# olegroshka/vae-channel-dynamics

Measured on AMD Instinct MI355X. Metric: images/sec SDXL-VAE train step @256x256 (tracking on), higher is better.
Workload: dtype f32

## Files before the change

### vae-channel-dynamics_amd/csrc/igemm.hip

```cpp
#include "bf16_frag.h"
#include <algorithm>
#include <stdlib.h>
#include <type_traits>

#include "launchers.h"

namespace {

struct LanePos {
  int lr, lh, trq, trp, trh;
};
__device__ __forceinline__ LanePos lane_pos(int lane) { return LanePos{lane & 31, lane >> 5, (lane & 15) >> 2, lane & 3, (lane >> 4) & 1}; }

struct F32 {
  typedef float elem;
  typedef f32x4 raw4;
  typedef f32x4 frag;
  typedef unsigned off_t;
  static constexpr int BK_ROWS = 32, BK_WGRAD = 32;
  static constexpr int KG = 8;
  static constexpr int PAD_K = 4, PAD_T = 4;
  static constexpr bool SETPRIO = true;
  static constexpr bool PAIR16 = false;
  static constexpr bool flag(int32_t) { return false; }

  static __device__ __forceinline__ raw4 load4(__amdgpu_buffer_rsrc_t rs, unsigned, bool ok, int row, int ld, int c) {
    return VAE_BUF_LOAD4(rs, oob_unless(ok, ((unsigned)row * (unsigned)ld + (unsigned)c) * 4u));
  }
  static __device__ __forceinline__ f32x4 to_f32(raw4 r, bool) { return r; }
  static __device__ __forceinline__ void put4(elem* d, f32x4 v) { *reinterpret_cast<f32x4*>(d) = v; }
  static __device__ __forceinline__ void put4_stored(elem* d, raw4, f32x4 v, bool) { put4(d, v); }
  static __device__ __forceinline__ frag frag_k(const elem* p) { return *reinterpret_cast<const f32x4*>(p); }
  static __device__ __forceinline__ frag frag_t(const elem* tile, int ld, int kg, LanePos l, int col0) {
    frag v;
#pragma unroll
    for (int j = 0; j < 4; ++j) v[j] = tile[(kg * 8 + l.lh * 4 + j) * ld + col0 + l.lr];
    return v;
  }
  template <int MI, int NI>
  static __device__ __forceinline__ void frags_tt(frag* a, frag* b, const elem* sA, int ldA, int colA, const elem* sB, int ldB, int colB, int kg, LanePos l) {
#pragma unroll
    for (int j = 0; j < 4; ++j) {
      const int k = kg * 8 + l.lh * 4 + j;
#pragma unroll
      for (int mi = 0; mi < MI; ++mi) a[mi][j] = sA[k * ldA + colA + mi * 32 + l.lr];
#pragma unroll
      for (int ni = 0; ni < NI; ++ni) b[ni][j] = sB[k * ldB + colB + ni * 32 + l.lr];
    }
  }
  template <int MI, int NI>
  static __device__ __forceinline__ void mma(f32x16 (&acc)[MI][NI], const frag* a, const frag* b) {
#pragma unroll
    for (int j = 0; j < 4; ++j)
#pragma unroll
      for (int mi = 0; mi < MI; ++mi)
#pragma unroll
        for (int ni = 0; ni < NI; ++ni) acc[mi][ni] = __builtin_amdgcn_mfma_f32_32x32x2f32(a[mi][j], b[ni][j], acc[mi][ni], 0, 0, 0);
  }
  static __device__ __forceinline__ off_t out_off(bool ok, int orow, int ldc, int col) {
    return ok ? ((unsigned)orow * (unsigned)ldc + (unsigned)col) * 4u : BUF_OOB;
  }
  static __device__ __forceinline__ bool inside(off_t o) { return o != BUF_OOB; }
  static __device__ __forceinline__ float load1(__amdgpu_buffer_rsrc_t rs, bool, off_t o) {
    return __builtin_bit_cast(float, __builtin_amdgcn_raw_buffer_load_b32(rs, o, 0, 0));
  }
  static __device__ __forceinline__ void store1(__amdgpu_buffer_rsrc_t rs, bool, off_t o, float v) {
    __builtin_amdgcn_raw_buffer_store_b32(__builtin_bit_cast(unsigned, v), rs, o, 0, 0);
  }
};

struct BF16 {
  typedef u16 elem;
  typedef uint4 raw4;
  typedef bf16x8 frag;
  typedef int off_t;
  static constexpr int BK_ROWS = 64, BK_WGRAD = 32;
  static constexpr int KG = 16;
  static constexpr int PAD_K = 8, PAD_T = 32;
  static constexpr bool SETPRIO = false;
  static constexpr bool PAIR16 = true;
  static __device__ __forceinline__ bool flag(int32_t v) { return v != 0; }

  static __device__ __forceinline__ raw4 load4(__amdgpu_buffer_rsrc_t rs, unsigned esize, bool ok, int row, int ld, int c) {
    return buf_load4_raw(rs, esize, neg_unless(ok, row * ld + c));
  }
  static __device__ __forceinline__ f32x4 to_f32(raw4 r, bool bf) { return raw4_to_f32(r, bf); }
  static __device__ __forceinline__ void put4(elem* d, f32x4 v) { *reinterpret_cast<uint2*>(d) = pack4(v); }
  static __device__ __forceinline__ void put4_stored(elem* d, raw4 r, f32x4 v, bool bf) {
    *reinterpret_cast<uint2*>(d) = bf ? uint2{r.x, r.y} : pack4(v);
  }
  static __device__ __forceinline__ frag frag_k(const elem* p) { return frag_direct(p); }
  static __device__ __forceinline__ frag frag_t(const elem* tile, int ld, int kg, LanePos l, int col0) {
    return frag_tr(tile + (kg * 16 + l.lh * 8 + l.trq) * ld + col0 + l.trh * 16 + l.trp * 4, ld);
  }
  template <int MI, int NI>
  static __device__ __forceinline__ void frags_tt(frag* a, frag* b, const elem* sA, int ldA, int colA, const elem* sB, int ldB, int colB, int kg, LanePos l) {
#pragma unroll
    for (int mi = 0; mi < MI; ++mi) a[mi] = frag_t(sA, ldA, kg, l, colA + mi * 32);
#pragma unroll
    for (int ni = 0; ni < NI; ++ni) b[ni] = frag_t(sB, ldB, kg, l, colB + ni * 32);
  }
  template <int MI, int NI>
  static __device__ __forceinline__ void mma(f32x16 (&acc)[MI][NI], const frag* a, const frag* b) {
#pragma unroll
    for (int mi = 0; mi < MI; ++mi)
#pragma unroll
      for (int ni = 0; ni < NI; ++ni) acc[mi][ni] = __builtin_amdgcn_mfma_f32_32x32x16_bf16(a[mi], b[ni], acc[mi][ni], 0, 0, 0);
  }
  static __device__ __forceinline__ off_t out_off(bool ok, int orow, int ldc, int col) { return ok ? orow * ldc + col : -1; }
  static __device__ __forceinline__ bool inside(off_t o) { return o >= 0; }
  static __device__ __forceinline__ float load1(__amdgpu_buffer_rsrc_t rs, bool bf, off_t o) { return buf_load1_elem(rs, bf, o); }
  static __device__ __forceinline__ void store1(__amdgpu_buffer_rsrc_t rs, bool bf, off_t o, float v) { buf_store1_elem(rs, bf, o, v); }

  static __device__ __forceinline__ bool pair16(const vae_igemm_args& p, bool cbf, bool rbf, const char* C) {
    return cbf && (p.N % 2 == 0) && (p.ldc % 2 == 0) && (p.res == nullptr || rbf) && p.track == nullptr && ((reinterpret_cast<uintptr_t>(C) & 3u) == 0);
  }
  template <int MI, int NI, class RowPixel>
  static __device__ __forceinline__ void store_pairs(const vae_igemm_args& p, const f32x16 (&acc)[MI][NI], int ni, __amdgpu_buffer_rsrc_t rsC,
                                                     __amdgpu_buffer_rsrc_t rsR, int col, bool colok, int m0, int trow0, int lh, bool s2c,
                                                     RowPixel row_pixel) {
    const bool odd = col & 1;
    const float b0 = (p.bias && colok) ? p.bias[col & ~1] : 0.f, b1 = (p.bias && colok) ? p.bias[col | 1] : 0.f;
#pragma unroll
    for (int mi = 0; mi < MI; ++mi) {
      unsigned o16[8], rr[8];
#pragma unroll
      for (int j = 0; j < 8; ++j) {
        const int r = 2 * j + (odd ? 1 : 0);
        const int row = trow0 + mi * 32 + (r & 3) + 8 * (r >> 2) + 4 * lh;
        int orow = row;
        if (s2c) {
          int b, y, x;
          row_pixel(row < p.M ? row : m0, b, y, x);
          orow = (b * p.g.Ho + y) * p.g.Wo + x;
        }
        o16[j] = (colok && row < p.M) ? (unsigned)(orow * p.ldc + (col & ~1)) * 2u : BUF_OOB;
        rr[j] = 0u;
      }
      if (p.res) {
#pragma unroll
        for (int j = 0; j < 8; ++j) rr[j] = __builtin_amdgcn_raw_buffer_load_b32(rsR, o16[j], 0, 0);
      }
#pragma unroll
      for (int j = 0; j < 8; ++j) {
        const float a0 = p.alpha * acc[mi][ni][2 * j], a1 = p.alpha * acc[mi][ni][2 * j + 1];
        const float recv = lane_xor1(odd ? a0 : a1);
        typedef __bf16 bf16x2_t __attribute__((ext_vector_type(2)));
        bf16x2_t h;
        h[0] = (__bf16)((odd ? recv : a0) + b0 + __builtin_bit_cast(float, rr[j] << 16));
        h[1] = (__bf16)((odd ? a1 : recv) + b1 + __builtin_bit_cast(float, rr[j] & 0xffff0000u));
        __builtin_amdgcn_raw_buffer_store_b32(__builtin_bit_cast(unsigned, h), rsC, o16[j], 0, 0);
      }
    }
  }
};

template <int MI, int NI>
__device__ __forceinline__ void zero_acc(f32x16 (&acc)[MI][NI]) {
#pragma unroll
  for (int mi = 0; mi < MI; ++mi)
#pragma unroll
    for (int ni = 0; ni < NI; ++ni)
#pragma unroll
      for (int r = 0; r < 16; ++r) acc[mi][ni][r] = 0.f;
}

template <class P, int BM, int BN, int WM, int WN, bool BKM, bool VEC, int XF>
__device__ __forceinline__ void rows_body(const vae_igemm_args& p) {
  typedef typename P::elem elem;
  constexpr int BK = P::BK_ROWS;
  constexpr int NT = 64 * WM * WN;
  constexpr int KQ = BK / 4;
  constexpr int RP = NT / KQ;
  constexpr int LDA = BK + P::PAD_K;
  constexpr int LDB = BKM ? (BN + P::PAD_T) : (BK + P::PAD_K);
  constexpr int SA = BM * LDA;
  constexpr int SB = BKM ? BK * LDB : BN * LDB;
  constexpr int STAGE = SA + SB;
  constexpr int SS = (XF != VAE_XF_NONE) ? 2 * SS_HALF * (4 / (int)sizeof(elem)) : 0;
  constexpr int TM = BM / WM, TN = BN / WN, MI = TM / 32, NI = TN / 32;
  constexpr int AR = BM / RP;
  constexpr int NQ = BN / 4, KR = NT / NQ;
  constexpr int BR = BKM ? (BK / KR) : (BN / RP);
  static_assert(AR >= 1 && BR >= 1 && TM % 32 == 0 && TN % 32 == 0 && (BK / P::KG == 2 || BK / P::KG == 4), "tile/wave layout");
  __shared__ __attribute__((aligned(16))) elem smem[2 * STAGE + SS];
  float* sS = reinterpret_cast<float*>(smem + 2 * STAGE);

  const int tid = threadIdx.x, lane = tid & 63, wave = tid >> 6;
  const int wm = wave / WN, wn = wave % WN;
  const LanePos lp = lane_pos(lane);
  const int lr = lp.lr, lh = lp.lh;
  const int tilesN = (p.N + BN - 1) / BN;
  const int tm = blockIdx.x / tilesN, tn = blockIdx.x % tilesN;
  const int m0 = tm * BM, n0 = tn * BN;
  const int z = blockIdx.z;
  const vae_conv_geom g = p.g;
  const SrcMap smap = make_srcmap(g);
  const bool abf = P::flag(p.a_bf16), cbf = P::flag(p.out_bf16), rbf = P::flag(p.res_bf16);
  const unsigned esA = abf ? 2u : 4u;
  const char* __restrict__ A = reinterpret_cast<const char*>(p.A) + (int64_t)z * p.sAb * esA;
  const float* __restrict__ W = p.W + (int64_t)z * p.sWb;
  const int hw = g.Ho * g.Wo;

  const bool s2c = (g.mode == VAE_MODE_DGRAD_S2);
  const int hh = g.Ho >> 1, wh = g.Wo >> 1;
  const int cls_rows = s2c ? p.M >> 2 : 1;
  const int cls = s2c ? m0 / cls_rows : 0;
  const int cpy = cls >> 1, cpx = cls & 1;
  const int nkw = s2c ? (cpx ? 1 : 2) : 3;
  const int ntaps = s2c ? (cpy ? 1 : 2) * nkw : g.taps;
  auto row_pixel = [&](int m, int& b, int& y, int& x) {
    if (s2c) {
      const int r = m - cls * cls_rows;
      b = r / (hh * wh);
      const int rem = r - b * (hh * wh);
      const int i = rem / wh;
      y = 2 * i + cpy;
      x = 2 * (rem - i * wh) + cpx;
    } else {
      b = m / hw;
      const int rem = m - b * hw;
      y = rem / g.Wo;
      x = rem - y * g.Wo;
    }
  };

  const int b_base = s2c ? (m0 - cls * cls_rows) / (hh * wh) : m0 / hw;
  const size_t img = (size_t)g.Hs * g.Ws * g.Cs;
  const size_t abytes = (size_t)(g.B - b_base) * img * esA, wbytes = (size_t)(BKM ? (int64_t)p.K * p.sk : (int64_t)p.N * p.sn) * 4u;
  const auto rsA = VAE_BUF_RSRC(A + (int64_t)b_base * img * esA, abytes < BUF_MAX ? abytes : BUF_MAX);
  const auto rsW = VAE_BUF_RSRC(W, wbytes < BUF_MAX ? wbytes : BUF_MAX);

  const int k4 = tid % KQ, r0 = tid / KQ;
  const int n4 = tid % NQ, kq = tid / NQ;
  int rb[AR], ry[AR], rx[AR];
#pragma unroll
  for (int i = 0; i < AR; ++i) {
    const int m = m0 + r0 + RP * i;
    if (m < p.M) {
      row_pixel(m, rb[i], ry[i], rx[i]);
    } else {
      rb[i] = -1; ry[i] = 0; rx[i] = 0;
    }
  }

  const int b_lo = m0 / hw;
  if (XF != VAE_XF_NONE) {
    const int b_hi = (min(p.M, m0 + BM) - 1) / hw;
    const int nent = min((b_hi - b_lo + 1) * p.K, SS_HALF);
    for (int i = tid; i < nent; i += NT) {
      const int j = i / p.K, c = i - j * p.K;
      sS[i] = p.scale[(int64_t)(b_lo + j) * g.Cs + c];
      sS[SS_HALF + i] = p.shift[(int64_t)(b_lo + j) * g.Cs + c];
    }
  }

  f32x16 acc[MI][NI];
  zero_acc(acc);

  const int kchunks = (p.K + BK - 1) / BK;
  const int steps = ntaps * kchunks;

  typename P::raw4 ra[AR];
  f32x4 rw[BR];
  int a_b[AR];
  int reg_c0 = 0;

  auto load_regs = [&](int s) {
    const int ord = s / kchunks;
    const int c0 = (s - ord * kchunks) * BK;
    reg_c0 = c0;
    int kh, kw;
    if (s2c) {
      const int a = ord / nkw;
      kh = cpy ? 1 : 2 * a;
      kw = cpx ? 1 : 2 * (ord - a * nkw);
    } else {
      kh = (g.taps == 9) ? ord / 3 : 0;
      kw = (g.taps == 9) ? ord - kh * 3 : 0;
    }
    const int tap = kh * 3 + kw;
    const int c = c0 + k4 * 4;
#pragma unroll
    for (int i = 0; i < AR; ++i) {
      int sy = 0, sx = 0;
      const bool ok = src_pixel(smap, ry[i], rx[i], kh, kw, sy, sx) && (rb[i] >= 0);
      if constexpr (VEC) ra[i] = P::load4(rsA, esA, ok && c < p.K, ((rb[i] - b_base) * g.Hs + sy) * g.Ws + sx, g.Cs, c);
      else ra[i] = load4s(p.A + (int64_t)z * p.sAb + (((int64_t)rb[i] * g.Hs + sy) * g.Ws + sx) * g.Cs + c, ok, c, p.K);
      a_b[i] = ok ? rb[i] : -1;
    }
    if (!BKM) {
#pragma unroll
      for (int i = 0; i < BR; ++i) {
        const int n = n0 + r0 + RP * i;
        if constexpr (VEC) rw[i] = VAE_BUF_LOAD4(rsW, oob_unless(n < p.N && c < p.K, ((unsigned)n * (unsigned)p.sn + (unsigned)tap * (unsigned)p.st + (unsigned)c) * 4u));
        else rw[i] = load4s(W + (int64_t)n * p.sn + (int64_t)tap * p.st + c, n < p.N, c, p.K);
      }
    } else {
#pragma unroll
      for (int i = 0; i < BR; ++i) {
        const int k = c0 + kq + KR * i;
        const int n = n0 + n4 * 4;
        if constexpr (VEC) rw[i] = VAE_BUF_LOAD4(rsW, oob_unless(k < p.K && n < p.N, ((unsigned)k * (unsigned)p.sk + (unsigned)tap * (unsigned)p.st + (unsigned)n) * 4u));
        else rw[i] = load4s(W + (int64_t)k * p.sk + (int64_t)tap * p.st + n, k < p.K, n, p.N);
      }
    }
  };
  auto store_lds = [&](elem* sA, elem* sB) {
    const int c = reg_c0 + k4 * 4;
#pragma unroll
    for (int i = 0; i < AR; ++i) {
      f32x4 v = P::to_f32(ra[i], abf);
      if (XF != VAE_XF_NONE) {
        const bool ok = (a_b[i] >= 0) && (c < p.K);
        const int o = ok ? (a_b[i] - b_lo) * p.K + c : 0;
        v = xform4_tab<XF>(v, sS + o, sS + SS_HALF + o, ok);
      }
      P::put4(&sA[(r0 + RP * i) * LDA + k4 * 4], v);
    }
#pragma unroll
    for (int i = 0; i < BR; ++i) {
      if (!BKM) P::put4(&sB[(r0 + RP * i) * LDB + k4 * 4], rw[i]);
      else P::put4(&sB[(kq + KR * i) * LDB + n4 * 4], rw[i]);
    }
  };
  typename P::frag fa[2][MI], fb[2][NI];
  auto fetch = [&](const elem* sA, const elem* sB, int kg, typename P::frag* a, typename P::frag* b) {
#pragma unroll
    for (int mi = 0; mi < MI; ++mi) a[mi] = P::frag_k(&sA[(wm * TM + mi * 32 + lr) * LDA + kg * P::KG + lh * (P::KG / 2)]);
#pragma unroll
    for (int ni = 0; ni < NI; ++ni) {
      if (!BKM) b[ni] = P::frag_k(&sB[(wn * TN + ni * 32 + lr) * LDB + kg * P::KG + lh * (P::KG / 2)]);
      else b[ni] = P::frag_t(sB, LDB, kg, lp, wn * TN + ni * 32);
    }
  };
  constexpr int NKG = BK / P::KG;
  auto compute = [&](const elem* sA, const elem* sB, int kg) {
    if (kg + 1 < NKG) fetch(sA, sB, kg + 1, fa[(kg + 1) & 1], fb[(kg + 1) & 1]);
    __builtin_amdgcn_sched_barrier(0);
    if (P::SETPRIO) __builtin_amdgcn_s_setprio(1);
    P::mma(acc, fa[kg & 1], fb[kg & 1]);
    if (P::SETPRIO) __builtin_amdgcn_s_setprio(0);
    __builtin_amdgcn_sched_barrier(0);
  };
  load_regs(0);
  __syncthreads();
  store_lds(smem, smem + SA);
  if (steps > 1) load_regs(1);
  __syncthreads();
  for (int s = 0; s < steps; ++s) {
    const elem* cA = smem + (s & 1) * STAGE;
    const elem* cB = cA + SA;
    fetch(cA, cB, 0, fa[0], fb[0]);
    compute(cA, cB, 0);
    if (NKG == 4) compute(cA, cB, 1);
    if (s + 1 < steps) {
      elem* nA = smem + ((s + 1) & 1) * STAGE;
      store_lds(nA, nA + SA);
      if (s + 2 < steps) load_regs(s + 2);
    }
    compute(cA, cB, NKG / 2);
    if (NKG == 4) compute(cA, cB, 3);
    __syncthreads();
  }

  const unsigned esC = cbf ? 2u : 4u, esR = rbf ? 2u : 4u;
  char* __restrict__ C = reinterpret_cast<char*>(p.C) + (int64_t)z * p.sCb * esC;
  const auto rsC = VAE_BUF_RSRC(C, (size_t)p.M * p.ldc * esC);
  const auto rsR = VAE_BUF_RSRC(p.res ? reinterpret_cast<const char*>(p.res) + (int64_t)z * p.sCb * esR : C, (size_t)p.M * p.ldc * (p.res ? esR : esC));
  float tsum[NI];
#pragma unroll
  for (int ni = 0; ni < NI; ++ni) tsum[ni] = 0.f;
  bool pair16 = false;
  if constexpr (P::PAIR16) pair16 = P::pair16(p, cbf, rbf, C);
#pragma unroll
  for (int ni = 0; ni < NI; ++ni) {
    const int col = n0 + wn * TN + ni * 32 + lr;
    const bool colok = col < p.N;
    const float bv = (p.bias && colok) ? p.bias[col] : 0.f;
    if constexpr (P::PAIR16) {
      if (pair16) {
        P::store_pairs(p, acc, ni, rsC, rsR, col, colok, m0, m0 + wm * TM, lh, s2c, row_pixel);
        continue;
      }
    }
#pragma unroll
    for (int mi = 0; mi < MI; ++mi) {
      typename P::off_t off[16];
      float rv[16];
#pragma unroll
      for (int r = 0; r < 16; ++r) {
        const int row = m0 + wm * TM + mi * 32 + (r & 3) + 8 * (r >> 2) + 4 * lh;
        int orow = row;
        if (s2c) {
          int b, y, x;
          row_pixel(row < p.M ? row : m0, b, y, x);
          orow = (b * g.Ho + y) * g.Wo + x;
        }
        off[r] = P::out_off(colok && row < p.M, orow, p.ldc, col);
        rv[r] = 0.f;
      }
      if (p.res) {
#pragma unroll
        for (int r = 0; r < 16; ++r) rv[r] = P::load1(rsR, rbf, off[r]);
      }
#pragma unroll
      for (int r = 0; r < 16; ++r) {
        const float v = p.alpha * acc[mi][ni][r] + bv + rv[r];
        P::store1(rsC, cbf, off[r], v);
        tsum[ni] += P::inside(off[r]) ? fabsf(v) : 0.f;
      }
    }
  }
  if (p.track && z == 0) {
    float* red = reinterpret_cast<float*>(smem);
#pragma unroll
    for (int ni = 0; ni < NI; ++ni) {
      const float s2 = tsum[ni] + __shfl_xor(tsum[ni], 32, 64);
      if (lh == 0) red[wm * BN + wn * TN + ni * 32 + lr] = s2;
    }
    __syncthreads();
    if (tid < BN) {
      float t = 0.f;
#pragma unroll
      for (int w = 0; w < WM; ++w) t += red[w * BN + tid];
      if (n0 + tid < p.N) p.track[(int64_t)tm * p.N + n0 + tid] = t;
    }
  }
}

template <class P, int BM, int BN, int WM, int WN, bool VEC, int XF>
__device__ __forceinline__ void wgrad_body(const vae_wgrad_args& p) {
  typedef typename P::elem elem;
  constexpr int BK = P::BK_WGRAD;
  constexpr int NT = 64 * WM * WN;
  constexpr int LDA = BM + P::PAD_T, LDB = BN + P::PAD_T;
  constexpr int SA = BK * LDA, SB = BK * LDB;
  constexpr int STAGE = SA + SB;
  constexpr int SS = (XF != VAE_XF_NONE) ? 2 * SS_HALF * (4 / (int)sizeof(elem)) : 0;
  constexpr int TM = BM / WM, TN = BN / WN, MI = TM / 32, NI = TN / 32;
  constexpr int AQ = BM / 4, AKR = NT / AQ, AI = BK / AKR;
  constexpr int BQ = BN / 4, BKR = NT / BQ, BI = BK / BKR;
  static_assert(AI >= 1 && BI >= 1 && TM % 32 == 0 && TN % 32 == 0 && (BK / P::KG == 2 || BK / P::KG == 4), "tile/wave layout");
  __shared__ __attribute__((aligned(16))) elem smem[2 * STAGE + SS];
  float* sS = reinterpret_cast<float*>(smem + 2 * STAGE);

  const int tid = threadIdx.x, lane = tid & 63, wave = tid >> 6;
  const int wm = wave / WN, wn = wave % WN;
  const LanePos lp = lane_pos(lane);
  const int lr = lp.lr, lh = lp.lh;
  const int tilesN = (p.N + BN - 1) / BN;
  const int tm = blockIdx.x / tilesN, tn = blockIdx.x % tilesN;
  const int m0 = tm * BM, n0 = tn * BN;
  const int tap = blockIdx.y / p.nsplit, split = blockIdx.y % p.nsplit;
  const int z = blockIdx.z;
  const vae_conv_geom g = p.g;
  const SrcMap smap = make_srcmap(g);
  const int kh = (g.taps == 9) ? tap / 3 : 0, kw = (g.taps == 9) ? tap - kh * 3 : 0;
  const bool ybf = P::flag(p.y_bf16), xbf = P::flag(p.x_bf16);
  const unsigned esY = ybf ? 2u : 4u, esX = xbf ? 2u : 4u;
  const char* __restrict__ dY = reinterpret_cast<const char*>(p.dY) + (int64_t)z * p.sYb * esY;
  const char* __restrict__ X = reinterpret_cast<const char*>(p.X) + (int64_t)z * p.sXb * esX;

  int chunk = (p.npix + p.nsplit - 1) / p.nsplit;
  chunk = ((chunk + 31) / 32) * 32;
  const int pbeg = split * chunk;
  const int pend = min(p.npix, pbeg + chunk);
  const int steps = (pend > pbeg) ? (pend - pbeg + BK - 1) / BK : 0;
  const int hw = g.Ho * g.Wo;
  const bool do_bias = (p.bias_partial != nullptr) && tn == 0 && tap == 0 && z == 0;

  const int b_lo = pbeg / hw;
  if (XF != VAE_XF_NONE && steps > 0) {
    const int nb = (pend - 1) / hw - b_lo + 1;
    const int ncol = min(BN, p.N - n0);
    const int nent = min(nb * BN, SS_HALF);
    for (int i = tid; i < nent; i += NT) {
      const int j = i / BN, c = i - j * BN;
      const bool ok = c < ncol;
      sS[i] = ok ? p.scale[(int64_t)(b_lo + j) * g.Cs + n0 + c] : 0.f;
      sS[SS_HALF + i] = ok ? p.shift[(int64_t)(b_lo + j) * g.Cs + n0 + c] : 0.f;
    }
  }

  f32x16 acc[MI][NI];
  zero_acc(acc);

  const size_t img = (size_t)g.Hs * g.Ws * g.Cs;
  const size_t ybytes = (size_t)(steps > 0 ? pend - pbeg : 0) * p.ldy * esY, xbytes = (size_t)(g.B - b_lo) * img * esX;
  const auto rsY = VAE_BUF_RSRC(dY + (int64_t)pbeg * p.ldy * esY, ybytes < BUF_MAX ? ybytes : BUF_MAX);
  const auto rsX = VAE_BUF_RSRC(X + (int64_t)b_lo * img * esX, xbytes < BUF_MAX ? xbytes : BUF_MAX);

  const int a4 = tid % AQ, akq = tid / AQ;
  const int b4 = tid % BQ, bkq = tid / BQ;
  typename P::raw4 ra[AI], rx[BI];
  int xb[BI];
  f32x4 bsum = {0.f, 0.f, 0.f, 0.f};

  auto load_regs = [&](int s) {
    const int pb = pbeg + s * BK;
#pragma unroll
    for (int i = 0; i < AI; ++i) {
      const int pix = pb + akq + AKR * i;
      const int c = m0 + a4 * 4;
      if constexpr (VEC) ra[i] = P::load4(rsY, esY, pix < pend && c < p.M, pix - pbeg, p.ldy, c);
      else ra[i] = load4s(p.dY + (int64_t)z * p.sYb + (int64_t)pix * p.ldy + c, pix < pend, c, p.M);
    }
#pragma unroll
    for (int i = 0; i < BI; ++i) {
      const int pix = pb + bkq + BKR * i;
      const int c = n0 + b4 * 4;
      const int b = pix / hw, rem = pix - b * hw;
      const int y = rem / g.Wo, x = rem - y * g.Wo;
      int sy = 0, sx = 0;
      const bool ok = src_pixel(smap, y, x, kh, kw, sy, sx) && (pix < pend);
      if constexpr (VEC) rx[i] = P::load4(rsX, esX, ok && c < p.N, ((b - b_lo) * g.Hs + sy) * g.Ws + sx, g.Cs, c);
      else rx[i] = load4s(p.X + (int64_t)z * p.sXb + (((int64_t)b * g.Hs + sy) * g.Ws + sx) * g.Cs + c, ok, c, p.N);
      xb[i] = ok ? b : -1;
    }
  };
  auto store_lds = [&](elem* sA, elem* sB) {
#pragma unroll
    for (int i = 0; i < AI; ++i) {
      const f32x4 v = P::to_f32(ra[i], ybf);
      P::put4_stored(&sA[(akq + AKR * i) * LDA + a4 * 4], ra[i], v, ybf);
      if (do_bias) bsum += v;
    }
#pragma unroll
    for (int i = 0; i < BI; ++i) {
      f32x4 v = P::to_f32(rx[i], xbf);
      if (XF != VAE_XF_NONE) {
        const bool ok = xb[i] >= 0;
        const int o = ok ? (xb[i] - b_lo) * BN + b4 * 4 : 0;
        v = xform4_tab<XF>(v, sS + o, sS + SS_HALF + o, ok);
      }
      P::put4(&sB[(bkq + BKR * i) * LDB + b4 * 4], v);
    }
  };
  typename P::frag fa[2][MI], fb[2][NI];
  auto fetch = [&](const elem* sA, const elem* sB, int kg, typename P::frag* a, typename P::frag* b) {
    P::template frags_tt<MI, NI>(a, b, sA, LDA, wm * TM, sB, LDB, wn * TN, kg, lp);
  };
  constexpr int NKG = BK / P::KG;
  auto compute = [&](const elem* sA, const elem* sB, int kg) {
    if (kg + 1 < NKG) fetch(sA, sB, kg + 1, fa[(kg + 1) & 1], fb[(kg + 1) & 1]);
    __builtin_amdgcn_sched_barrier(0);
    if (P::SETPRIO) __builtin_amdgcn_s_setprio(1);
    P::mma(acc, fa[kg & 1], fb[kg & 1]);
    if (P::SETPRIO) __builtin_amdgcn_s_setprio(0);
    __builtin_amdgcn_sched_barrier(0);
  };
  if (steps > 0) {
    load_regs(0);
    __syncthreads();
    store_lds(smem, smem + SA);
    if (steps > 1) load_regs(1);
    __syncthreads();
    for (int s = 0; s < steps; ++s) {
      const elem* cA = smem + (s & 1) * STAGE;
      const elem* cB = cA + SA;
      fetch(cA, cB, 0, fa[0], fb[0]);
      compute(cA, cB, 0);
      if (NKG == 4) compute(cA, cB, 1);
      if (s + 1 < steps) {
        elem* nA = smem + ((s + 1) & 1) * STAGE;
        store_lds(nA, nA + SA);
        if (s + 2 < steps) load_regs(s + 2);
      }
      compute(cA, cB, NKG / 2);
      if (NKG == 4) compute(cA, cB, 3);
      __syncthreads();
    }
  }

  const int64_t ld = (int64_t)g.taps * p.N;
  float* __restrict__ O = (p.nsplit == 1 ? p.out : p.partial + (int64_t)split * p.M * ld) + (int64_t)z * p.sOb;
#pragma unroll
  for (int ni = 0; ni < NI; ++ni) {
    const int col = n0 + wn * TN + ni * 32 + lr;
    if (col >= p.N) continue;
#pragma unroll
    for (int mi = 0; mi < MI; ++mi)
#pragma unroll
      for (int r = 0; r < 16; ++r) {
        const int row = m0 + wm * TM + mi * 32 + (r & 3) + 8 * (r >> 2) + 4 * lh;
        if (row < p.M) O[(int64_t)row * ld + (int64_t)tap * p.N + col] = p.alpha * acc[mi][ni][r];
      }
  }
  if (do_bias) {
    f32x4* red = reinterpret_cast<f32x4*>(smem);
    red[akq * AQ + a4] = bsum;
    __syncthreads();
    if (tid < AQ) {
      f32x4 t = {0.f, 0.f, 0.f, 0.f};
      for (int r = 0; r < AKR; ++r) t += red[r * AQ + tid];
#pragma unroll
      for (int e = 0; e < 4; ++e) {
        const int m = m0 + tid * 4 + e;
        if (m < p.M) p.bias_partial[(int64_t)split * p.M + m] = t[e];
      }
    }
  }
}

template <int BM, int BN, int WM, int WN, bool BKM, bool VEC, int XF>
__global__ __launch_bounds__(64 * WM * WN) void igemm_rows_kernel(vae_igemm_args p) { rows_body<F32, BM, BN, WM, WN, BKM, VEC, XF>(p); }
template <int BM, int BN, int WM, int WN, bool VEC, int XF>
__global__ __launch_bounds__(64 * WM * WN) void wgrad_kernel(vae_wgrad_args p) { wgrad_body<F32, BM, BN, WM, WN, VEC, XF>(p); }
template <int BM, int BN, int WM, int WN, bool BKM, int XF>
__global__ __launch_bounds__(64 * WM * WN) void igemm_rows_bf16_kernel(vae_igemm_args p) { rows_body<BF16, BM, BN, WM, WN, BKM, true, XF>(p); }
template <int BM, int BN, int WM, int WN, int XF>
__global__ __launch_bounds__(64 * WM * WN) void wgrad_bf16_kernel(vae_wgrad_args p) { wgrad_body<BF16, BM, BN, WM, WN, true, XF>(p); }

__device__ __forceinline__ void small_column_sums(const float* __restrict__ partial2, int nsplit, int n2, float* __restrict__ out2, int blk) {
  const int i = blk * 256 + (int)threadIdx.x;
  if (i >= n2) return;
  const float* p = partial2 + i;
  float s = 0.f;
  int k = 0;
  for (; k + 16 <= nsplit; k += 16) {
    float v[16];
#pragma unroll
    for (int j = 0; j < 16; ++j) v[j] = p[(int64_t)(k + j) * n2];
#pragma unroll
    for (int j = 0; j < 16; ++j) s += v[j];
  }
  for (; k < nsplit; ++k) s += p[(int64_t)k * n2];
  out2[i] = s;
}

template <int KP>
__global__ __launch_bounds__(256) void reduce_splits_kernel(const float* __restrict__ partial, int nsplit, int64_t n, float* __restrict__ out,
                                                            int main_blocks, const float* __restrict__ partial2, int n2, float* __restrict__ out2) {
  constexpr int COLS = 256 / KP;
  __shared__ f32x4 red[KP > 1 ? 256 : 1];
  if ((int)blockIdx.x >= main_blocks) {
    small_column_sums(partial2, nsplit, n2, out2, (int)blockIdx.x - main_blocks);
    return;
  }
  const int col = threadIdx.x % COLS, kp = threadIdx.x / COLS;
  const int64_t n4 = n >> 2;
  const int per = (nsplit + KP - 1) / KP;
  const int k0 = kp * per, k1 = min(nsplit, k0 + per);
  auto column = [&](int64_t i) {
    f32x4 s = {0.f, 0.f, 0.f, 0.f};
    const f32x4* p = reinterpret_cast<const f32x4*>(partial) + i;
    int k = k0;
    for (; k + 8 <= k1; k += 8) {
      f32x4 v[8];
#pragma unroll
      for (int j = 0; j < 8; ++j) v[j] = p[(int64_t)(k + j) * n4];
      s += ((v[0] + v[1]) + (v[2] + v[3])) + ((v[4] + v[5]) + (v[6] + v[7]));
    }
    for (; k < k1; ++k) s += p[(int64_t)k * n4];
    return s;
  };
  if (KP == 1) {
    for (int64_t i = (int64_t)blockIdx.x * 256 + threadIdx.x; i < n4; i += (int64_t)main_blocks * 256) reinterpret_cast<f32x4*>(out)[i] = column(i);
    return;
  }
  const int64_t i = (int64_t)blockIdx.x * COLS + col;
  f32x4 s = {0.f, 0.f, 0.f, 0.f};
  if (i < n4) s = column(i);
  red[threadIdx.x] = s;
  __syncthreads();
  if (kp == 0 && i < n4) {
#pragma unroll
    for (int j = 1; j < KP; ++j) s += red[j * COLS + col];
    reinterpret_cast<f32x4*>(out)[i] = s;
  }
}
__global__ void reduce_splits_scalar_kernel(const float* __restrict__ partial, int nsplit, int64_t n, float* __restrict__ out) {
  int64_t i = (int64_t)blockIdx.x * blockDim.x + threadIdx.x;
  const int64_t stride = (int64_t)gridDim.x * blockDim.x;
  for (; i < n; i += stride) {
    float s = 0.f;
    for (int k = 0; k < nsplit; ++k) s += partial[(int64_t)k * n + i];
    out[i] = s;
  }
}

template <int NPOS, int TCI>
__global__ __launch_bounds__(256) void wgrad_wino_reduce_kernel(const float* __restrict__ slab, int nsplit, int N, int M, float* __restrict__ dW,
                                                                int tiles, const float* __restrict__ bpart, float* __restrict__ db) {
  constexpr int TQ = 8, TCO = 4 * TQ, Q = TCI * TQ, KP = 256 / Q, NP = (NPOS + KP - 1) / KP;
  constexpr int ST0 = KP > 1 ? NPOS * Q * 4 : 0;
  __shared__ __attribute__((aligned(16))) float smem[ST0 + 9 * TCO * (TCI + 1)];
  const int tid = threadIdx.x;
  if ((int)blockIdx.x >= tiles) {
    small_column_sums(bpart, nsplit, M, db, (int)blockIdx.x - tiles);
    return;
  }
  const int tilesM = M / TCO;
  const int c0 = ((int)blockIdx.x / tilesM) * TCI, m0 = ((int)blockIdx.x % tilesM) * TCO;
  const int q = tid % Q, kp = tid / Q;
  const int cq = q % TQ, cl = q / TQ;
  const int64_t pstride4 = ((int64_t)N * M) >> 2, sstride4 = NPOS * pstride4;
  const f32x4* src = reinterpret_cast<const f32x4*>(slab + (int64_t)(c0 + cl) * M + m0 + 4 * cq);
  const f32x4* sp[NP];
#pragma unroll
  for (int j = 0; j < NP; ++j) sp[j] = src + (kp + j * KP < NPOS ? kp + j * KP : 0) * pstride4;
  auto tree8 = [](const f32x4* v) { return ((v[0] + v[1]) + (v[2] + v[3])) + ((v[4] + v[5]) + (v[6] + v[7])); };
  auto range = [&](int k0, int k1, f32x4(&g)[NP]) {
#pragma unroll
    for (int j = 0; j < NP; ++j) g[j] = f32x4{0.f, 0.f, 0.f, 0.f};
    int k = k0;
    if constexpr (NP == 1) {
      for (; k + 16 <= k1; k += 16) {
        f32x4 v[16];
#pragma unroll
        for (int i = 0; i < 16; ++i) v[i] = sp[0][(int64_t)(k + i) * sstride4];
        g[0] += tree8(v);
        g[0] += tree8(v + 8);
      }
    }
    for (; k + 8 <= k1; k += 8) {
#pragma unroll
      for (int j = 0; j < NP; ++j) {
        f32x4 v[8];
#pragma unroll
        for (int i = 0; i < 8; ++i) v[i] = sp[j][(int64_t)(k + i) * sstride4];
        g[j] += tree8(v);
      }
    }
    for (; k < k1; ++k) {
      f32x4 v[NP];
#pragma unroll
      for (int j = 0; j < NP; ++j) v[j] = sp[j][(int64_t)k * sstride4];
#pragma unroll
      for (int j = 0; j < NP; ++j) g[j] += v[j];
    }
  };
  f32x4 mine[NP];
  if (nsplit >= 32) {
    const int per = (nsplit + 3) / 4;
    range(0, min(nsplit, per), mine);
    for (int r = 1; r < 4; ++r) {
      f32x4 g[NP];
      range(r * per, min(nsplit, (r + 1) * per), g);
#pragma unroll
      for (int j = 0; j < NP; ++j) mine[j] += g[j];
    }
  } else {
    range(0, nsplit, mine);
  }
  f32x4 acc[NPOS];
  if constexpr (KP > 1) {
    f32x4* red = reinterpret_cast<f32x4*>(smem);
#pragma unroll
    for (int j = 0; j < NP; ++j)
      if (kp + j * KP < NPOS) red[(kp + j * KP) * Q + q] = mine[j];
    __syncthreads();
    if (kp == 0) {
#pragma unroll
      for (int p = 0; p < NPOS; ++p) acc[p] = red[p * Q + q];
    }
  } else {
#pragma unroll
    for (int p = 0; p < NPOS; ++p) acc[p] = mine[p];
  }
  float(*sT)[TCO][TCI + 1] = reinterpret_cast<float(*)[TCO][TCI + 1]>(smem + ST0);
  if (kp == 0) {
    f32x4 o[9];
    if constexpr (NPOS == 16) {
      f32x4 h[3][4];
#pragma unroll
      for (int j = 0; j < 4; ++j) {
        const float cj = (j == 1 || j == 2) ? 0.5f : 1.f;
        const f32x4 r0 = acc[0 * 4 + j] * cj, r1 = acc[1 * 4 + j] * (0.5f * cj), r2 = acc[2 * 4 + j] * (0.5f * cj), r3 = acc[3 * 4 + j] * cj;
        h[0][j] = (r0 + r1) + r2;
        h[1][j] = r1 - r2;
        h[2][j] = (r1 + r2) - r3;
      }
#pragma unroll
      for (int a = 0; a < 3; ++a) {
        o[a * 3 + 0] = (h[a][0] + h[a][1]) + h[a][2];
        o[a * 3 + 1] = h[a][1] - h[a][2];
        o[a * 3 + 2] = (h[a][1] + h[a][2]) - h[a][3];
      }
    } else {
      f32x4 h[3][3];
#pragma unroll
      for (int j = 0; j < 3; ++j) {
        h[0][j] = acc[0 * 3 + j] + acc[1 * 3 + j];
        h[1][j] = acc[1 * 3 + j];
        h[2][j] = acc[1 * 3 + j] - acc[2 * 3 + j];
      }
#pragma unroll
      for (int a = 0; a < 3; ++a) {
        o[a * 3 + 0] = h[a][0] + h[a][1];
        o[a * 3 + 1] = h[a][1];
        o[a * 3 + 2] = h[a][1] - h[a][2];
      }
    }
#pragma unroll
    for (int t = 0; t < 9; ++t)
#pragma unroll
      for (int e = 0; e < 4; ++e) sT[t][4 * cq + e][cl] = o[t][e];
  }
  __syncthreads();
  for (int idx = tid; idx < 9 * TCO * TCI; idx += 256) {
    const int c = idx % TCI, r = idx / TCI;
    const int t = r % 9, ml = r / 9;
    dW[((int64_t)(m0 + ml) * 9 + t) * N + c0 + c] = sT[t][ml][c];
  }
}

template <int V>
using int_c = std::integral_constant<int, V>;
using std::false_type;
using std::true_type;

template <class Launch>
bool dispatch_xf(int xf, Launch launch) {
  switch (xf) {
    case VAE_XF_NONE: launch(int_c<VAE_XF_NONE>{}); return true;
    case VAE_XF_AFFINE: launch(int_c<VAE_XF_AFFINE>{}); return true;
    case VAE_XF_AFFINE_SILU: launch(int_c<VAE_XF_AFFINE_SILU>{}); return true;
    default: return false;
  }
}

template <bool BF, int BM, int BN, int WM, int WN>
int launch_rows_tile(const vae_igemm_args& a, bool bkm, bool vec, hipStream_t st) {
// ... 117 lines not shown
```

Measured before the change: 108.2.

## Stage f32 transposed GEMM tiles k-major in LDS and step load counters incrementally

For the f32 path, the weight tile in the forward implicit GEMM and both tiles in the weight-gradient kernel are now stored k-major in LDS. MFMA fragments can then be read with one 16-byte LDS load instead of four scalar reads. Per-step address math (tap decode, pixel coordinates) is replaced by incremental counters and precomputed row offsets, with the per-step weight and dY offsets passed as scalar soffset values. The cost is a scatter-style transposed LDS write (four scalar stores per vector) and more complex indexing with new static layout constraints.

```diff
diff --git a/vae-channel-dynamics_amd/csrc/igemm.hip b/vae-channel-dynamics_amd/csrc/igemm.hip
--- a/vae-channel-dynamics_amd/csrc/igemm.hip
+++ b/vae-channel-dynamics_amd/csrc/igemm.hip
@@ -20,9 +20,14 @@
   static constexpr int BK_ROWS = 32, BK_WGRAD = 32;
   static constexpr int KG = 8;
   static constexpr int PAD_K = 4, PAD_T = 4;
+  static constexpr bool T_KMAJOR = true;
+  static constexpr int T_KLANES = 16;
+  static constexpr bool STEP_COUNTERS = true;
   static constexpr bool SETPRIO = true;
   static constexpr bool PAIR16 = false;
   static constexpr bool flag(int32_t) { return false; }
+  static constexpr unsigned off_unit(unsigned) { return 4u; }
+  static __device__ __forceinline__ raw4 load4_off(__amdgpu_buffer_rsrc_t rs, unsigned, bool ok, unsigned off) { return VAE_BUF_LOAD4(rs, oob_unless(ok, off)); }
 
   static __device__ __forceinline__ raw4 load4(__amdgpu_buffer_rsrc_t rs, unsigned, bool ok, int row, int ld, int c) {
     return VAE_BUF_LOAD4(rs, oob_unless(ok, ((unsigned)row * (unsigned)ld + (unsigned)c) * 4u));
@@ -31,22 +36,19 @@
   static __device__ __forceinline__ void put4(elem* d, f32x4 v) { *reinterpret_cast<f32x4*>(d) = v; }
   static __device__ __forceinline__ void put4_stored(elem* d, raw4, f32x4 v, bool) { put4(d, v); }
   static __device__ __forceinline__ frag frag_k(const elem* p) { return *reinterpret_cast<const f32x4*>(p); }
+  static __device__ __forceinline__ void put4_t(elem* tile, int ld, int k, int col, f32x4 v) {
+#pragma unroll
+    for (int e = 0; e < 4; ++e) tile[(col + e) * ld + k] = v[e];
+  }
   static __device__ __forceinline__ frag frag_t(const elem* tile, int ld, int kg, LanePos l, int col0) {
-    frag v;
-#pragma unroll
-    for (int j = 0; j < 4; ++j) v[j] = tile[(kg * 8 + l.lh * 4 + j) * ld + col0 + l.lr];
-    return v;
+    return frag_k(&tile[(col0 + l.lr) * ld + kg * 8 + l.lh * 4]);
   }
   template <int MI, int NI>
   static __device__ __forceinline__ void frags_tt(frag* a, frag* b, const elem* sA, int ldA, int colA, const elem* sB, int ldB, int colB, int kg, LanePos l) {
 #pragma unroll
-    for (int j = 0; j < 4; ++j) {
-      const int k = kg * 8 + l.lh * 4 + j;
-#pragma unroll
-      for (int mi = 0; mi < MI; ++mi) a[mi][j] = sA[k * ldA + colA + mi * 32 + l.lr];
-#pragma unroll
-      for (int ni = 0; ni < NI; ++ni) b[ni][j] = sB[k * ldB + colB + ni * 32 + l.lr];
-    }
+    for (int mi = 0; mi < MI; ++mi) a[mi] = frag_t(sA, ldA, kg, l, colA + mi * 32);
+#pragma unroll
+    for (int ni = 0; ni < NI; ++ni) b[ni] = frag_t(sB, ldB, kg, l, colB + ni * 32);
   }
   template <int MI, int NI>
   static __device__ __forceinline__ void mma(f32x16 (&acc)[MI][NI], const frag* a, const frag* b) {
@@ -77,9 +79,16 @@
   static constexpr int BK_ROWS = 64, BK_WGRAD = 32;
   static constexpr int KG = 16;
   static constexpr int PAD_K = 8, PAD_T = 32;
+  static constexpr bool T_KMAJOR = false;
+  static constexpr int T_KLANES = 16;
+  static constexpr bool STEP_COUNTERS = false;
   static constexpr bool SETPRIO = false;
   static constexpr bool PAIR16 = true;
   static __device__ __forceinline__ bool flag(int32_t v) { return v != 0; }
+  static constexpr unsigned off_unit(unsigned) { return 1u; }
+  static __device__ __forceinline__ raw4 load4_off(__amdgpu_buffer_rsrc_t rs, unsigned esize, bool ok, unsigned off) {
+    return buf_load4_raw(rs, esize, neg_unless(ok, (int)off));
+  }
 
   static __device__ __forceinline__ raw4 load4(__amdgpu_buffer_rsrc_t rs, unsigned esize, bool ok, int row, int ld, int c) {
     return buf_load4_raw(rs, esize, neg_unless(ok, row * ld + c));
@@ -89,6 +98,7 @@
   static __device__ __forceinline__ void put4_stored(elem* d, raw4 r, f32x4 v, bool bf) {
     *reinterpret_cast<uint2*>(d) = bf ? uint2{r.x, r.y} : pack4(v);
   }
+  static __device__ __forceinline__ void put4_t(elem* tile, int ld, int k, int col, f32x4 v) { put4(&tile[k * ld + col], v); }
   static __device__ __forceinline__ frag frag_k(const elem* p) { return frag_direct(p); }
   static __device__ __forceinline__ frag frag_t(const elem* tile, int ld, int kg, LanePos l, int col0) {
     return frag_tr(tile + (kg * 16 + l.lh * 8 + l.trq) * ld + col0 + l.trh * 16 + l.trp * 4, ld);
@@ -165,6 +175,12 @@
       for (int r = 0; r < 16; ++r) acc[mi][ni][r] = 0.f;
 }
 
+__device__ __forceinline__ bool src_pixel_t(const SrcMap& m, int ty, int tx, int& sy, int& sx) {
+  sy = ty >> m.sh;
+  sx = tx >> m.sh;
+  return ((unsigned)ty < m.limy) & ((unsigned)tx < m.limx) & (((ty | tx) & m.pm) == 0) & ((unsigned)sy < (unsigned)m.Hs) & ((unsigned)sx < (unsigned)m.Ws);
+}
+
 template <class P, int BM, int BN, int WM, int WN, bool BKM, bool VEC, int XF>
 __device__ __forceinline__ void rows_body(const vae_igemm_args& p) {
   typedef typename P::elem elem;
@@ -173,15 +189,18 @@
   constexpr int KQ = BK / 4;
   constexpr int RP = NT / KQ;
   constexpr int LDA = BK + P::PAD_K;
-  constexpr int LDB = BKM ? (BN + P::PAD_T) : (BK + P::PAD_K);
+  constexpr bool TK = BKM && P::T_KMAJOR;
+  constexpr int LDB = (BKM && !TK) ? (BN + P::PAD_T) : (BK + P::PAD_K);
   constexpr int SA = BM * LDA;
-  constexpr int SB = BKM ? BK * LDB : BN * LDB;
+  constexpr int SB = (BKM && !TK) ? BK * LDB : BN * LDB;
   constexpr int STAGE = SA + SB;
   constexpr int SS = (XF != VAE_XF_NONE) ? 2 * SS_HALF * (4 / (int)sizeof(elem)) : 0;
   constexpr int TM = BM / WM, TN = BN / WN, MI = TM / 32, NI = TN / 32;
   constexpr int AR = BM / RP;
   constexpr int NQ = BN / 4, KR = NT / NQ;
   constexpr int BR = BKM ? (BK / KR) : (BN / RP);
+  constexpr int NW = NT / 64;
+  static_assert(!TK || (BK == 32 && NW % (32 / P::T_KLANES) == 0 && BR * NW * 2 == NQ), "k-major staging of the n-contiguous weight tile");
   static_assert(AR >= 1 && BR >= 1 && TM % 32 == 0 && TN % 32 == 0 && (BK / P::KG == 2 || BK / P::KG == 4), "tile/wave layout");
   __shared__ __attribute__((aligned(16))) elem smem[2 * STAGE + SS];
   float* sS = reinterpret_cast<float*>(smem + 2 * STAGE);
@@ -231,16 +250,42 @@
   const auto rsA = VAE_BUF_RSRC(A + (int64_t)b_base * img * esA, abytes < BUF_MAX ? abytes : BUF_MAX);
   const auto rsW = VAE_BUF_RSRC(W, wbytes < BUF_MAX ? wbytes : BUF_MAX);
 
+  auto tap_kh = [&](int ta) { return s2c ? (cpy ? 1 : 2 * ta) : ta; };
+  auto tap_kw = [&](int tb) { return s2c ? (cpx ? 1 : 2 * tb) : tb; };
+  const bool lin = (smap.sh == 0) || s2c;
+  const int kh0 = tap_kh(0), kw0 = tap_kw(0);
+  const unsigned uA = P::off_unit(esA);
+
   const int k4 = tid % KQ, r0 = tid / KQ;
-  const int n4 = tid % NQ, kq = tid / NQ;
-  int rb[AR], ry[AR], rx[AR];
+  constexpr int KL = P::T_KLANES, QL = 64 / KL, KB = 32 / KL;
+  const int n4 = TK ? (lane / KL + QL * (wave / KB)) : tid % NQ, kq = TK ? ((wave % KB) * KL + lane % KL) : tid / NQ;
+  constexpr int N4P = TK ? QL * (NW / KB) : 0, KRP = TK ? 0 : KR;
+  int rb[AR], rty[AR], rtx[AR];
+  unsigned roff[AR];
 #pragma unroll
   for (int i = 0; i < AR; ++i) {
     const int m = m0 + r0 + RP * i;
-    if (m < p.M) {
-      row_pixel(m, rb[i], ry[i], rx[i]);
+    int y = 0, x = 0;
+    rb[i] = -1;
+    if (m < p.M) row_pixel(m, rb[i], y, x);
+    const int ty = y * smap.a + smap.cy, tx = x * smap.a + smap.cx;
+    const int sy = (ty + kh0 * smap.b) >> smap.sh, sx = (tx + kw0 * smap.b) >> smap.sh;
+    rty[i] = !P::STEP_COUNTERS ? y : (m < p.M) ? (lin ? sy : ty) : (int)0xC0000000;
+    rtx[i] = !P::STEP_COUNTERS ? x : lin ? sx : tx;
+    roff[i] = ((unsigned)((((rb[i] - b_base) * g.Hs + sy) * g.Ws + sx) * g.Cs) + (unsigned)(k4 * 4)) * uA;
+  }
+  unsigned woff[BR];
+  bool wok[BR];
+#pragma unroll
+  for (int i = 0; i < BR; ++i) {
+    if (!BKM) {
+      const int n = n0 + r0 + RP * i;
+      wok[i] = n < p.N;
+      woff[i] = ((unsigned)n * (unsigned)p.sn + (unsigned)(k4 * 4)) * 4u;
     } else {
-      rb[i] = -1; ry[i] = 0; rx[i] = 0;
+      const int n = n0 + (n4 + N4P * i) * 4;
+      wok[i] = n < p.N;
+      woff[i] = ((unsigned)(kq + KRP * i) * (unsigned)p.sk + (unsigned)n) * 4u;
     }
   }
 
@@ -265,45 +310,82 @@
   f32x4 rw[BR];
   int a_b[AR];
   int reg_c0 = 0;
+  int ld_c0 = 0, ld_ta = 0, ld_tb = 0;
 
   auto load_regs = [&](int s) {
-    const int ord = s / kchunks;
-    const int c0 = (s - ord * kchunks) * BK;
+    if constexpr (!P::STEP_COUNTERS) {
+      const int ord = s / kchunks;
+      const int c0 = (s - ord * kchunks) * BK;
+      reg_c0 = c0;
+      const int kh = tap_kh(ord / nkw), kw = tap_kw(ord - (ord / nkw) * nkw);
+      const int tap = kh * 3 + kw;
+      const int c = c0 + k4 * 4;
+#pragma unroll
+      for (int i = 0; i < AR; ++i) {
+        int sy = 0, sx = 0;
+        const bool ok = src_pixel(smap, rty[i], rtx[i], kh, kw, sy, sx) && (rb[i] >= 0);
+        ra[i] = P::load4(rsA, esA, ok && c < p.K, ((rb[i] - b_base) * g.Hs + sy) * g.Ws + sx, g.Cs, c);
+        a_b[i] = ok ? rb[i] : -1;
+      }
+#pragma unroll
+      for (int i = 0; i < BR; ++i) {
+        if (!BKM) {
+          const int n = n0 + r0 + RP * i;
+          rw[i] = VAE_BUF_LOAD4(rsW, oob_unless(n < p.N && c < p.K, ((unsigned)n * (unsigned)p.sn + (unsigned)tap * (unsigned)p.st + (unsigned)c) * 4u));
+        } else {
+          const int k = c0 + kq + KR * i, n = n0 + n4 * 4;
+          rw[i] = VAE_BUF_LOAD4(rsW, oob_unless(k < p.K && n < p.N, ((unsigned)k * (unsigned)p.sk + (unsigned)tap * (unsigned)p.st + (unsigned)n) * 4u));
+        }
+      }
+      return;
+    }
+    const int c0 = ld_c0, kh = tap_kh(ld_ta), kw = tap_kw(ld_tb);
     reg_c0 = c0;
-    int kh, kw;
-    if (s2c) {
-      const int a = ord / nkw;
-      kh = cpy ? 1 : 2 * a;
-      kw = cpx ? 1 : 2 * (ord - a * nkw);
-    } else {
-      kh = (g.taps == 9) ? ord / 3 : 0;
-      kw = (g.taps == 9) ? ord - kh * 3 : 0;
-    }
     const int tap = kh * 3 + kw;
     const int c = c0 + k4 * 4;
+    const bool cok = c < p.K;
+    const int dsy = ((kh - kh0) * smap.b) >> smap.sh, dsx = ((kw - kw0) * smap.b) >> smap.sh;
+    const unsigned dA = (unsigned)((dsy * g.Ws + dsx) * g.Cs + c0) * uA;
+    const int tkh = kh * smap.b, tkw = kw * smap.b;
+    int sy[AR], sx[AR];
+    bool ok[AR];
+    if (lin) {
+#pragma unroll
+      for (int i = 0; i < AR; ++i) {
+        sy[i] = rty[i] + dsy;
+        sx[i] = rtx[i] + dsx;
+        ok[i] = ((unsigned)sy[i] < (unsigned)g.Hs) & ((unsigned)sx[i] < (unsigned)g.Ws);
+        if constexpr (VEC) ra[i] = P::load4_off(rsA, esA, ok[i] & cok, roff[i] + dA);
+      }
+    } else {
+#pragma unroll
+      for (int i = 0; i < AR; ++i) {
+        ok[i] = src_pixel_t(smap, rty[i] + tkh, rtx[i] + tkw, sy[i], sx[i]);
+        if constexpr (VEC) ra[i] = P::load4(rsA, esA, ok[i] && cok, ((rb[i] - b_base) * g.Hs + sy[i]) * g.Ws + sx[i], g.Cs, c);
+      }
+    }
 #pragma unroll
     for (int i = 0; i < AR; ++i) {
-      int sy = 0, sx = 0;
-      const bool ok = src_pixel(smap, ry[i], rx[i], kh, kw, sy, sx) && (rb[i] >= 0);
-      if constexpr (VEC) ra[i] = P::load4(rsA, esA, ok && c < p.K, ((rb[i] - b_base) * g.Hs + sy) * g.Ws + sx, g.Cs, c);
-      else ra[i] = load4s(p.A + (int64_t)z * p.sAb + (((int64_t)rb[i] * g.Hs + sy) * g.Ws + sx) * g.Cs + c, ok, c, p.K);
-      a_b[i] = ok ? rb[i] : -1;
-    }
-    if (!BKM) {
-#pragma unroll
-      for (int i = 0; i < BR; ++i) {
-        const int n = n0 + r0 + RP * i;
-        if constexpr (VEC) rw[i] = VAE_BUF_LOAD4(rsW, oob_unless(n < p.N && c < p.K, ((unsigned)n * (unsigned)p.sn + (unsigned)tap * (unsigned)p.st + (unsigned)c) * 4u));
-        else rw[i] = load4s(W + (int64_t)n * p.sn + (int64_t)tap * p.st + c, n < p.N, c, p.K);
-      }
-    } else {
-#pragma unroll
-      for (int i = 0; i < BR; ++i) {
-        const int k = c0 + kq + KR * i;
-        const int n = n0 + n4 * 4;
-        if constexpr (VEC) rw[i] = VAE_BUF_LOAD4(rsW, oob_unless(k < p.K && n < p.N, ((unsigned)k * (unsigned)p.sk + (unsigned)tap * (unsigned)p.st + (unsigned)n) * 4u));
-        else rw[i] = load4s(W + (int64_t)k * p.sk + (int64_t)tap * p.st + n, k < p.K, n, p.N);
-      }
+      if constexpr (!VEC) ra[i] = load4s(p.A + (int64_t)z * p.sAb + (((int64_t)rb[i] * g.Hs + sy[i]) * g.Ws + sx[i]) * g.Cs + c, ok[i], c, p.K);
+      a_b[i] = ok[i] ? rb[i] : -1;
+    }
+    const unsigned wstep = __builtin_amdgcn_readfirstlane(((unsigned)tap * (unsigned)p.st + (unsigned)c0 * (BKM ? (unsigned)p.sk : 1u)) * 4u);
+#pragma unroll
+    for (int i = 0; i < BR; ++i) {
+      const bool ok = wok[i] && (BKM ? (c0 + kq + KRP * i < p.K) : cok);
+      if constexpr (VEC) {
+        rw[i] = __builtin_bit_cast(f32x4, __builtin_amdgcn_raw_buffer_load_b128(rsW, oob_unless(ok, woff[i]), wstep, 0));
+      } else if (!BKM) {
+        rw[i] = load4s(W + (int64_t)(n0 + r0 + RP * i) * p.sn + (int64_t)tap * p.st + c, wok[i], c, p.K);
+      } else {
+        const int k = c0 + kq + KRP * i, n = n0 + (n4 + N4P * i) * 4;
+        rw[i] = load4s(W + (int64_t)k * p.sk + (int64_t)tap * p.st + n, k < p.K, n, p.N);
+      }
+    }
+    ld_c0 += BK;
+    if (ld_c0 >= p.K) {
+      ld_c0 = 0;
+      if (++ld_tb == nkw) { ld_tb = 0; ++ld_ta; }
     }
   };
   auto store_lds = [&](elem* sA, elem* sB) {
@@ -321,7 +403,7 @@
 #pragma unroll
     for (int i = 0; i < BR; ++i) {
       if (!BKM) P::put4(&sB[(r0 + RP * i) * LDB + k4 * 4], rw[i]);
-      else P::put4(&sB[(kq + KR * i) * LDB + n4 * 4], rw[i]);
+      else P::put4_t(sB, LDB, kq + KRP * i, (n4 + N4P * i) * 4, rw[i]);
     }
   };
   typename P::frag fa[2][MI], fb[2][NI];
@@ -434,13 +516,16 @@
   typedef typename P::elem elem;
   constexpr int BK = P::BK_WGRAD;
   constexpr int NT = 64 * WM * WN;
-  constexpr int LDA = BM + P::PAD_T, LDB = BN + P::PAD_T;
-  constexpr int SA = BK * LDA, SB = BK * LDB;
+  constexpr bool TK = P::T_KMAJOR;
+  constexpr int LDA = TK ? BK + P::PAD_K : BM + P::PAD_T, LDB = TK ? BK + P::PAD_K : BN + P::PAD_T;
+  constexpr int SA = TK ? BM * LDA : BK * LDA, SB = TK ? BN * LDB : BK * LDB;
   constexpr int STAGE = SA + SB;
   constexpr int SS = (XF != VAE_XF_NONE) ? 2 * SS_HALF * (4 / (int)sizeof(elem)) : 0;
   constexpr int TM = BM / WM, TN = BN / WN, MI = TM / 32, NI = TN / 32;
   constexpr int AQ = BM / 4, AKR = NT / AQ, AI = BK / AKR;
   constexpr int BQ = BN / 4, BKR = NT / BQ, BI = BK / BKR;
+  constexpr int NW = NT / 64;
+  static_assert(!TK || (BK == 32 && NW % (32 / P::T_KLANES) == 0 && BI * NW * 2 == BQ), "k-major staging");
   static_assert(AI >= 1 && BI >= 1 && TM % 32 == 0 && TN % 32 == 0 && (BK / P::KG == 2 || BK / P::KG == 4), "tile/wave layout");
   __shared__ __attribute__((aligned(16))) elem smem[2 * STAGE + SS];
   float* sS = reinterpret_cast<float*>(smem + 2 * STAGE);
@@ -491,14 +576,66 @@
   const auto rsY = VAE_BUF_RSRC(dY + (int64_t)pbeg * p.ldy * esY, ybytes < BUF_MAX ? ybytes : BUF_MAX);
   const auto rsX = VAE_BUF_RSRC(X + (int64_t)b_lo * img * esX, xbytes < BUF_MAX ? xbytes : BUF_MAX);
 
-  const int a4 = tid % AQ, akq = tid / AQ;
+  static_assert(!TK || 64 % AKR == 0, "k-major staging: a wave holds whole pixel columns of dY");
+  const int a4 = TK ? lane / AKR + (64 / AKR) * wave : tid % AQ, akq = TK ? lane % AKR : tid / AQ;
   const int b4 = tid % BQ, bkq = tid / BQ;
   typename P::raw4 ra[AI], rx[BI];
   int xb[BI];
   f32x4 bsum = {0.f, 0.f, 0.f, 0.f};
 
+  constexpr int KL = P::T_KLANES, QL = 64 / KL, KB = 32 / KL;
+  const int tk = (wave % KB) * KL + lane % KL, tq = lane / KL + QL * (wave / KB);
+  constexpr int QP = QL * (NW / KB);
+  int wpix = pbeg + tk, wb = wpix / hw, wy = (wpix - wb * hw) / g.Wo, wx = wpix - wb * hw - wy * g.Wo;
+  const int d_b = BK / hw, d_y = (BK - d_b * hw) / g.Wo, d_x = BK - d_b * hw - d_y * g.Wo;
+  unsigned ystep = 0;
+  unsigned yoff[AI], xcol[BI];
+  bool yok[AI], xok[BI];
+  if constexpr (TK) {
+#pragma unroll
+    for (int i = 0; i < AI; ++i) {
+      yok[i] = m0 + a4 * 4 < p.M;
+      yoff[i] = ((unsigned)(akq + AKR * i) * (unsigned)p.ldy + (unsigned)(m0 + a4 * 4)) * 4u;
+    }
+#pragma unroll
+    for (int i = 0; i < BI; ++i) {
+      const int c = n0 + (tq + QP * i) * 4;
+      xok[i] = c < p.N;
+      xcol[i] = (unsigned)c * 4u;
+    }
+  }
+
   auto load_regs = [&](int s) {
     const int pb = pbeg + s * BK;
+    if constexpr (TK) {
+      int sy = 0, sx = 0;
+      const bool pok = wpix < pend;
+      const bool ok = src_pixel(smap, wy, wx, kh, kw, sy, sx) && pok;
+      const unsigned so = __builtin_amdgcn_readfirstlane(ystep);
+#pragma unroll
+      for (int i = 0; i < AI; ++i) {
+        const int pix = pb + akq + AKR * i;
+        if constexpr (VEC) ra[i] = __builtin_bit_cast(f32x4, __builtin_amdgcn_raw_buffer_load_b128(rsY, oob_unless(pix < pend && yok[i], yoff[i]), so, 0));
+        else ra[i] = load4s(p.dY + (int64_t)z * p.sYb + (int64_t)pix * p.ldy + m0 + a4 * 4, pix < pend, m0 + a4 * 4, p.M);
+      }
+      const unsigned xpix = (unsigned)((((wb - b_lo) * g.Hs + sy) * g.Ws + sx) * g.Cs) * 4u;
+#pragma unroll
+      for (int i = 0; i < BI; ++i) {
+        if constexpr (VEC) rx[i] = VAE_BUF_LOAD4(rsX, oob_unless(ok && xok[i], xpix + xcol[i]));
+        else rx[i] = load4s(p.X + (int64_t)z * p.sXb + (((int64_t)wb * g.Hs + sy) * g.Ws + sx) * g.Cs + n0 + (tq + QP * i) * 4, ok, n0 + (tq + QP * i) * 4, p.N);
+      }
+      xb[0] = ok ? wb : -1;
+      wpix += BK;
+      ystep += (unsigned)BK * (unsigned)p.ldy * 4u;
+      wx += d_x;
+      const int cx = wx >= g.Wo ? 1 : 0;
+      wx -= cx ? g.Wo : 0;
+      wy += d_y + cx;
+      const int cy = wy >= g.Ho ? 1 : 0;
+      wy -= cy ? g.Ho : 0;
+      wb += d_b + cy;
+      return;
+    }
 #pragma unroll
     for (int i = 0; i < AI; ++i) {
       const int pix = pb + akq + AKR * i;
@@ -520,6 +657,25 @@
     }
   };
   auto store_lds = [&](elem* sA, elem* sB) {
+    if constexpr (TK) {
+#pragma unroll
+      for (int i = 0; i < AI; ++i) {
+        const f32x4 v = P::to_f32(ra[i], ybf);
+        P::put4_t(sA, LDA, akq + AKR * i, a4 * 4, v);
+        if (do_bias) bsum += v;
+      }
+#pragma unroll
+      for (int i = 0; i < BI; ++i) {
+        f32x4 v = P::to_f32(rx[i], xbf);
+        if (XF != VAE_XF_NONE) {
+          const bool ok = xb[0] >= 0;
+          const int o = ok ? (xb[0] - b_lo) * BN + (tq + QP * i) * 4 : 0;
+          v = xform4_tab<XF>(v, sS + o, sS + SS_HALF + o, ok);
+        }
+        P::put4_t(sB, LDB, tk, (tq + QP * i) * 4, v);
+      }
+      return;
+    }
 #pragma unroll
     for (int i = 0; i < AI; ++i) {
       const f32x4 v = P::to_f32(ra[i], ybf);
```

Measured after the change: 108.8, median of 6. Within noise of the previous version (+0.6%).
